# djamahl99/findnpropagate

Hardware: AMD Instinct MI355X
Metric: NuScenes scenes/s (30k pts, Transfusion voxel backbone) (higher is better)
Workload: dtype bf16

## Files before the change

findnpropagate_amd/csrc/spconv.hip:

```cpp
#include "rankgrid.h"
#include "sortedsweep.h"
#include "conv_launch.h"
#include <type_traits>

#ifndef FNP_ABLATE
#define FNP_ABLATE 0
#endif

namespace {

__device__ __forceinline__ float to_f32(float v) { return v; }
__device__ __forceinline__ float to_f32(__bf16 v) { return (float)v; }
__device__ __forceinline__ float to_f32(_Float16 v) { return (float)v; }
template <typename T> __device__ __forceinline__ T from_f32(float v);
template <> __device__ __forceinline__ float from_f32<float>(float v) { return v; }
template <> __device__ __forceinline__ __bf16 from_f32<__bf16>(float v) { return (__bf16)v; }
template <> __device__ __forceinline__ _Float16 from_f32<_Float16>(float v) { return (_Float16)v; }

template <typename TIn, typename TOut>
__global__ __launch_bounds__(256) void spconv_valu_kernel(const TIn *__restrict__ x, const TIn *__restrict__ w,
                                                          const int *__restrict__ nbr, int nbr_stride, int K,
                                                          const int *__restrict__ n_out, int cap,
                                                          TOut *__restrict__ y, const float *__restrict__ scale,
                                                          const float *__restrict__ shift,
                                                          const TOut *__restrict__ residual, int relu, int Cin, int Cout) {
    const int n = min(*n_out, cap);
    const long long total = (long long)n * Cout;
    for (long long t = (long long)blockIdx.x * blockDim.x + threadIdx.x; t < total; t += (long long)gridDim.x * blockDim.x) {
        const int row = (int)(t / Cout), co = (int)(t % Cout);
        float acc = 0.f;
        for (int k = 0; k < K; ++k) {
            const int idx = nbr[(size_t)k * nbr_stride + row];
            if (idx < 0) continue;
            const TIn *xr = x + (size_t)idx * Cin;
            const TIn *wr = w + ((size_t)k * Cout + co) * Cin;
            for (int ci = 0; ci < Cin; ++ci) acc = fmaf(to_f32(xr[ci]), to_f32(wr[ci]), acc);
        }
        float v = acc;
        if (scale) v = v * scale[co] + shift[co];
        if (residual) v = v + to_f32(residual[(size_t)row * Cout + co]);
        if (relu && v < 0.f) v = 0.f;
        y[(size_t)row * Cout + co] = from_f32<TOut>(v);
    }
}

template <int COUT, typename TOut>
__global__ __launch_bounds__(256) void spconv_first_kernel(const float *__restrict__ x, const float *__restrict__ w,
                                                           const int *__restrict__ nbr, int nbr_stride, int K,
                                                           const int *__restrict__ n_out, int cap,
                                                           TOut *__restrict__ y, const float *__restrict__ scale,
                                                           const float *__restrict__ shift,
                                                           const TOut *__restrict__ residual, int relu, int Cin) {
    extern __shared__ __attribute__((aligned(16))) unsigned char fnp_smem[];
    float *wl = reinterpret_cast<float *>(fnp_smem);
    for (int i = threadIdx.x; i < K * Cin * COUT; i += 256) {
        const int k = i / (Cin * COUT), r = i % (Cin * COUT);
        const int ci = r / COUT, co = r % COUT;
        wl[i] = w[((size_t)k * COUT + co) * Cin + ci];
    }
    __syncthreads();
    const int n = min(*n_out, cap);
    for (int row = blockIdx.x * 256 + threadIdx.x; row < n; row += gridDim.x * 256) {
        float acc[COUT];
#pragma unroll
        for (int co = 0; co < COUT; ++co) acc[co] = 0.f;
        for (int k0 = 0; k0 < K; k0 += 9) {
            int idx[9];
#pragma unroll
            for (int j = 0; j < 9; ++j) idx[j] = k0 + j < K ? nbr[(size_t)(k0 + j) * nbr_stride + row] : -1;
#pragma unroll
            for (int j = 0; j < 9; ++j) {
                if (k0 + j >= K) break;
                const bool ok = idx[j] >= 0;
                const float *xr = x + (size_t)(ok ? idx[j] : 0) * Cin;
                const float *wk = wl + (k0 + j) * Cin * COUT;
                float xv[8];
#pragma unroll
                for (int ci = 0; ci < 8; ++ci) xv[ci] = ci < Cin ? xr[ci] : 0.f;
#pragma unroll
                for (int ci = 0; ci < 8; ++ci) {
                    if (ci >= Cin) break;
                    const float xc = ok ? xv[ci] : 0.f;
#pragma unroll
                    for (int co = 0; co < COUT; ++co) acc[co] = fmaf(xc, wk[ci * COUT + co], acc[co]);
                }
            }
        }
#pragma unroll
        for (int co = 0; co < COUT; ++co) {
            float v = acc[co];
            if (scale) v = v * scale[co] + shift[co];
            if (residual) v = v + to_f32(residual[(size_t)row * COUT + co]);
            if (relu && v < 0.f) v = 0.f;
            y[(size_t)row * COUT + co] = from_f32<TOut>(v);
        }
    }
}

template <typename TOut>
int launch_first(const ConvArgs &a, int Cin) {
    const int grid = fnp_grid_for(a.cap, 256, 2048);
    const size_t lds = sizeof(float) * (size_t)a.K * Cin * 16;
    hipLaunchKernelGGL(HIP_KERNEL_NAME(spconv_first_kernel<16, TOut>), dim3(grid), dim3(256), lds, a.stream, (const float *)a.x,
                       (const float *)a.w, a.nbr, a.nbr_stride, a.K, a.n_out, a.cap, (TOut *)a.y, a.scale, a.shift, (const TOut *)a.residual,
                       a.relu, Cin);
    FNP_LAUNCH_CHECK();
    return FNP_OK;
}

template <int CIN, int COUT, int KVOL>
struct MfmaCfg {
    static constexpr bool PAIR = CIN == 16 && KVOL == 27;
    static constexpr int KEFF = PAIR ? (KVOL + 1) / 2 : KVOL;
    static constexpr int CH = PAIR ? 4 : CIN / 8;
    static constexpr int SLAB = COUT * CH;
    static constexpr int SW = (CH == 8 || CH == 4) ? 1 : 0;
    static constexpr bool ALLK = KVOL > 0 && (long long)KEFF * SLAB * 16 <= 65536;
    static constexpr int LDS_BYTES = (ALLK ? KEFF : 2) * SLAB * 16;
    static constexpr int KS = (CIN + 31) / 32;
    static constexpr int PFK = ALLK ? (KS == 1 ? 4 : 2) : 1;
    static constexpr int WH = 64;
    static constexpr int WZERO = 128;
    static constexpr int win_rows(int nw, int mb) { return nw * mb * 16 + 2 * WH; }
    static constexpr bool WIDE = COUT >= 32;
    static constexpr int ESTRIDE = COUT * 2 + 16;
    static constexpr int epi_sites(bool win) { return win ? 8 : 16; }
    static constexpr int epi_bytes(int nw, bool win, bool out16) { return (WIDE && out16 && !win) ? nw * epi_sites(win) * ESTRIDE : 0; }
    static constexpr int lds_bytes(int nw, int mb, bool win) { return LDS_BYTES + (win ? win_rows(nw, mb) * CH * 16 + WZERO : 0); }
};

template <int CIN, int COUT> struct MfmaWg {
    static constexpr int NW = (CIN == COUT && CIN >= 32) ? 8 : 4;
    static constexpr int MB = COUT >= 128 ? 3 : (CIN == COUT || (CIN == 16 && COUT == 32)) ? 2 : 4;
    static constexpr int MB_SMALL = 2;
};

template <int CIN, int COUT> struct MfmaOcc { static constexpr int WAVES = (CIN == 128 && COUT == 128) ? 2 : (CIN == COUT || (CIN == 16 && COUT == 32)) ? 4 : (CIN < COUT && COUT <= 64) ? 3 : 2; };

struct FusedRb {
    RG gi;
    int s[3], p[3];
    const int *out_coords;
    const unsigned *ell_rec;
    int ell_cap;
};

struct SplitOut {
    const void *addend;
    void *hi, *lo;
    int relu;
};

#ifdef FNP_MFMA_STAMP
__device__ unsigned long long g_mfma_stamps[8];
#define FNP_MS_NOW(v) do { __builtin_amdgcn_sched_barrier(0); asm volatile("s_memtime %0\n\ts_waitcnt lgkmcnt(0)" : "=s"(v)::"memory"); __builtin_amdgcn_sched_barrier(0); } while (0)
#define FNP_MS(ph) do { if (CIN == 128 && COUT == 128 && KVOL == 27) { unsigned long long n_; FNP_MS_NOW(n_); ms_acc[ph] += n_ - ms_prev; ms_prev = n_; } } while (0)
#else
#define FNP_MS(ph)
#endif
template <int CIN, int COUT, int NWO> struct NwOf { static constexpr int value = NWO ? NWO : MfmaWg<CIN, COUT>::NW; };
template <int CIN, int COUT, int MB, int KVOL, bool WIN, typename TOut, bool FUSED = false, typename TAct = __bf16, bool SORTED = false, int NWO = 0>
__global__ __launch_bounds__((NwOf<CIN, COUT, NWO>::value * 64), (MfmaOcc<CIN, COUT>::WAVES)) void spconv_mfma_kernel(const TAct *__restrict__ x, int x_bytes,
                                                             const TAct *__restrict__ w,
                                                             const int *__restrict__ nbr, int nbr_stride, int Krt,
                                                             const int *__restrict__ n_out, int cap,
                                                             TOut *__restrict__ y, const float *__restrict__ scale,
                                                             const float *__restrict__ shift,
                                                             const TOut *__restrict__ residual, int relu, int hints, FusedRb frb, SortedRb srb, SplitOut so) {
    using Cfg = MfmaCfg<CIN, COUT, KVOL>;
    constexpr int NWX = NwOf<CIN, COUT, NWO>::value;
    static_assert(!SORTED || (KVOL == 27 && !WIN && !FUSED && !Cfg::PAIR && !Cfg::ALLK), "sorted sweep: wide double-buffered 3x3x3 layers");
    using bf16x8 = typename Vec16<TAct>::v8;
    using bf16x4 = typename Vec16<TAct>::v4;
    static_assert(sizeof(TOut) == 4 || std::is_same<TOut, TAct>::value, "16-bit outputs have the activation type");
    static_assert(!FUSED || (KVOL == 27 && !WIN), "fused rulebook: 3x3x3 strided layers");
    constexpr int CH = Cfg::CH, SLAB = Cfg::SLAB, SW = Cfg::SW, KS = Cfg::KS, PFK = Cfg::PFK;
    constexpr bool ALLK = Cfg::ALLK;
    constexpr int WROWS = Cfg::win_rows(NWX, MB), WH = Cfg::WH;
    static_assert(!WIN || (CH == 8 && PFK == 1), "window path: 64 input channels, fragments read one offset ahead");
    constexpr int NB = COUT / 16;
    constexpr int NBH = NB < 4 ? NB : 4;
    constexpr int ROWS_PER_WAVE = MB * 16;
    constexpr int NW = NWX, NT = NW * 64;
    constexpr int ROWS_PER_WG = NW * ROWS_PER_WAVE;
    constexpr int NCH = (SLAB + NT - 1) / NT;
    constexpr int WST = (NCH + KS - 1) / KS;
    constexpr bool WDEEP = !ALLK && NCH <= 1;
    constexpr bool WD4 = !ALLK && (((NW == 8 || (NW == 4 && CIN == 128 && COUT == 64)) && NCH == KS && NCH == 4) || (NWO == 4 && NCH == 2 * KS && KS == 4) ||
                                   (NW == 4 && NCH == 2 * KS && KS == 2 && CIN == 64 && COUT == 128));
    constexpr int WDN = WD4 ? NCH / KS : 1;
    static_assert(CIN % 16 == 0 && COUT % 16 == 0, "channel counts must be multiples of 16");
    static_assert(ALLK || SLAB % NT == 0 || SLAB < NT, "unsupported slab size");

    extern __shared__ __attribute__((aligned(16))) unsigned char fnp_smem[];
    uint4 *wl = reinterpret_cast<uint4 *>(fnp_smem);
    unsigned char *const win = fnp_smem + Cfg::LDS_BYTES;
    constexpr unsigned WIN_ZERO = (unsigned)(Cfg::LDS_BYTES + WROWS * CH * 16);
    auto win_sw = [](unsigned d) -> unsigned { return (d >> 1) & 7u; };

    constexpr bool PAIR = Cfg::PAIR;
    constexpr bool GPAIR = !WIN && KS % 2 == 0 && PFK == 1;
    const int K = KVOL > 0 ? Cfg::KEFF : Krt;
    const int n = min(*n_out, cap);
    const int tid = threadIdx.x;
    const int lane = tid & 63, wave = tid >> 6;
    const int l15 = lane & 15, q = lane >> 4;
    const bool kvalid0 = PAIR || (q * 8) < CIN;
    const int qk = PAIR ? (q >> 1) : 0;

    const __amdgpu_buffer_rsrc_t xrsrc = __builtin_amdgcn_make_buffer_rsrc((void *)x, 0, x_bytes, 0x00020000);
    auto row_off = [&](int id) -> unsigned {
        return ((FNP_ABLATE & 1) || id < 0 || !kvalid0) ? 0x80000000u
                                                        : (unsigned)id * (unsigned)(CIN * 2) + (unsigned)(PAIR ? (q & 1) : q) * 16u;
    };
    auto gather = [&](unsigned roff, int ks) -> bf16x8 {
        u32x4 v = {0u, 0u, 0u, 0u};
        if (!(WIN && (FNP_ABLATE & 8))) v = __builtin_amdgcn_raw_buffer_load_b128(xrsrc, roff + (unsigned)ks * 64u, 0, 0);
        return *reinterpret_cast<bf16x8 *>(&v);
    };
    constexpr int SR = MB * 16;
    int *const fstrip = reinterpret_cast<int *>(fnp_smem + Cfg::lds_bytes(NWX, MB, WIN) +
                                                Cfg::epi_bytes(NWX, WIN, sizeof(TOut) == 2)) + wave * (27 * SR);
    int frow0 = 0;
    float *const ss_lds = reinterpret_cast<float *>(fnp_smem + Cfg::lds_bytes(NWX, MB, WIN) +
                                                    Cfg::epi_bytes(NWX, WIN, sizeof(TOut) == 2) +
                                                    (FUSED ? NWX * 27 * MB * 16 * 4 : 0));
    auto nbr_at = [&](int k, int r, int r_end) -> int {
        const int rc = r < r_end ? r : r_end - 1;
        const int kr = PAIR ? 2 * k + qk : k, KR = PAIR ? KVOL : K;
        const int kc = kr < KR ? kr : KR - 1;
        if constexpr (FUSED) return kr < KR ? fstrip[kc * SR + (r - frow0)] : -1;
        const int v = nbr[(FNP_ABLATE & 32) ? (size_t)((kc * 64 + rc) & 0x3fff) : (size_t)kc * nbr_stride + rc];
        return (r < r_end && kr < KR) ? v : -1;
    };
    auto nbr_raw = [&](int k, int r, int r_end) -> int {
        const int rc = r < r_end ? r : r_end - 1;
        const int kr = PAIR ? 2 * k + qk : k, KR = PAIR ? KVOL : K;
        const int kc = kr < KR ? kr : KR - 1;
        if (FNP_ABLATE & 512) return rc + kc - 13;
        if constexpr (FUSED) return fstrip[kc * SR + (r - frow0)];
        return nbr[(FNP_ABLATE & 32) ? (size_t)((kc * 64 + rc) & 0x3fff) : (size_t)kc * nbr_stride + rc];
    };
    auto k_live = [&](int k) -> bool { return PAIR ? (2 * k + qk < KVOL) : (k < K); };

    auto win_off = [&](int id, int wlo) -> unsigned {
        if (FNP_ABLATE & 64)
            return (unsigned)Cfg::LDS_BYTES + ((((unsigned)id << 6) & 0x3fc0u) ^ ((unsigned)q << 4));
        const unsigned d = (unsigned)(id - wlo);
        return d < (unsigned)WROWS ? (unsigned)Cfg::LDS_BYTES + ((d * CH + ((unsigned)q ^ win_sw(d))) << 4) : WIN_ZERO;
    };
    auto row_off_w = [&](int id, int wlo) -> unsigned {
        const unsigned d = (unsigned)(id - wlo);
        return ((FNP_ABLATE & 1) || id < 0 || d < (unsigned)WROWS) ? 0x80000000u
                                                                    : (unsigned)id * (unsigned)(CIN * 2) + (unsigned)q * 16u;
    };
    auto win_read = [&](unsigned off) -> u32x4 {
        if (FNP_ABLATE & 16) return u32x4{off, 0u, 0u, 0u};
        return *reinterpret_cast<const u32x4 *>(fnp_smem + off);
    };

    const int G = gridDim.x;
    const int xcd = blockIdx.x & 7, slot = blockIdx.x >> 3;
    const int per = G >> 3, rem = G & 7;
    const int range = (xcd < rem ? xcd * (per + 1) : rem * (per + 1) + (xcd - rem) * per) + slot;
    int row_begin, row_end;
    int xslots = 1;
    if constexpr (SORTED) {
        const XcdRows xr = fnp_xcd_rows(n, G, xcd);
        row_begin = xr.X0;
        row_end = xr.X1;
        xslots = xr.S;
    } else {
        fnp_range_rows(n, range, G, row_begin, row_end);
    }
    if (row_begin >= row_end) return;
    for (int c = tid; c < 2 * COUT; c += NWX * 64)
        ss_lds[c] = scale ? (c < COUT ? scale[c] : shift[c - COUT]) : (c < COUT ? 1.f : 0.f);

#define FNP_LDS_POS(row, chunk) ((row) * CH + ((chunk) ^ (((row) >> SW) & (CH - 1))))
    int aoff[KS];
#pragma unroll
    for (int ks = 0; ks < KS; ++ks) aoff[ks] = FNP_LDS_POS(l15, kvalid0 ? ks * 4 + q : (q & (CH - 1)));
    const int st_pos0 = FNP_LDS_POS(tid / CH, tid % CH);
    static_assert(SLAB < NT || ((NT / CH) % (CH << SW) == 0), "staging swizzle must be periodic in NT chunks");
    if (WIN && tid < Cfg::WZERO / 16) reinterpret_cast<uint4 *>(fnp_smem + WIN_ZERO)[tid] = make_uint4(0u, 0u, 0u, 0u);
    if (ALLK) {
        for (int p = tid; p < K * SLAB; p += NT) {
            const int kk = p / SLAB, r = p % SLAB;
            if constexpr (PAIR) {
                const int co = r / CH, c = r % CH, kr = 2 * kk + (c >> 1);
                uint4 v = make_uint4(0u, 0u, 0u, 0u);
                if (kr < KVOL) v = reinterpret_cast<const uint4 *>(w)[((size_t)kr * COUT + co) * 2 + (c & 1)];
                wl[kk * SLAB + FNP_LDS_POS(co, c)] = v;
            } else {
                wl[kk * SLAB + FNP_LDS_POS(r / CH, r % CH)] = reinterpret_cast<const uint4 *>(w)[p];
            }
        }
        __syncthreads();
    }

#ifdef FNP_MFMA_STAMP
    unsigned long long ms_acc[4] = {0, 0, 0, 0}, ms_prev;
    FNP_MS_NOW(ms_prev);
#endif
    bool first_tile = true;
// ... 379 lines not shown
                            *slot = bf16x4{(TAct)v[0], (TAct)v[1], (TAct)v[2], (TAct)v[3]};
                        }
                    }
#pragma unroll
                    for (int i = 0; i < NRD; ++i) {
                        const int r = rb + i * SPI + wsite;
                        int ro = r;
                        if constexpr (SORTED) ro = orow[mb][h][i];
                        const u32x4 t = *reinterpret_cast<const u32x4 *>(eb + (i * SPI + wsite) * ES + wchunk * 16);
                        if (r < row_end && !(FNP_ABLATE & 128)) {
                            *reinterpret_cast<u32x4 *>(y + (size_t)ro * COUT + wchunk * 8) = t;
                        }
                    }
                }
            }
        } else if constexpr (WIN && sizeof(TOut) == 2 && NB % 2 == 0) {
            const int poff = (q & 1) * 32 + (q >> 1) * 16;
#pragma unroll
            for (int mb = 0; mb < MBT; ++mb) {
                const int r = row0 + mb * 16 + l15;
                const bool live = r < row_end;
#pragma unroll
                for (int kp = 0; kp < NB / 2; ++kp) {
                    uint2 ra = make_uint2(0u, 0u), rb = make_uint2(0u, 0u);
                    if (residual && !(FNP_ABLATE & 256)) {
                        uint4 rv = make_uint4(0u, 0u, 0u, 0u);
                        if (live) rv = *reinterpret_cast<const uint4 *>(reinterpret_cast<const unsigned char *>(residual) + (size_t)r * (COUT * 2) + kp * 64 + poff);
                        auto t0 = __builtin_amdgcn_permlane16_swap(rv.x, rv.z, false, false);
                        auto t1 = __builtin_amdgcn_permlane16_swap(rv.y, rv.w, false, false);
                        ra = make_uint2(t0[0], t1[0]);
                        rb = make_uint2(t0[1], t1[1]);
                    }
                    uint2 o[2];
#pragma unroll
                    for (int h = 0; h < 2; ++h) {
                        const int nb = 2 * kp + h, c0 = nb * 16 + q * 4;
                        float v[4];
#pragma unroll
                        for (int j = 0; j < 4; ++j) v[j] = acc[nb][mb][j];
                        if (scale) {
                            const float4 s4 = *reinterpret_cast<const float4 *>(ss_lds + c0);
                            const float4 h4 = *reinterpret_cast<const float4 *>(ss_lds + COUT + c0);
                            v[0] = v[0] * s4.x + h4.x; v[1] = v[1] * s4.y + h4.y; v[2] = v[2] * s4.z + h4.z; v[3] = v[3] * s4.w + h4.w;
                        }
                        if (residual && !(FNP_ABLATE & 256)) {
                            const uint2 rr = h ? rb : ra;
                            const bf16x4 t = *reinterpret_cast<const bf16x4 *>(&rr);
#pragma unroll
                            for (int j = 0; j < 4; ++j) v[j] = v[j] + (float)t[j];
                        }
                        if (relu) {
#pragma unroll
                            for (int j = 0; j < 4; ++j) v[j] = v[j] < 0.f ? 0.f : v[j];
                        }
                        const bf16x4 ob = {(TAct)v[0], (TAct)v[1], (TAct)v[2], (TAct)v[3]};
                        o[h] = *reinterpret_cast<const uint2 *>(&ob);
                    }
                    auto t0 = __builtin_amdgcn_permlane16_swap(o[0].x, o[1].x, false, false);
                    auto t1 = __builtin_amdgcn_permlane16_swap(o[0].y, o[1].y, false, false);
                    if (live && !(FNP_ABLATE & 128))
                        *reinterpret_cast<uint4 *>(reinterpret_cast<unsigned char *>(y) + (size_t)r * (COUT * 2) + kp * 64 + poff) =
                            make_uint4(t0[0], t1[0], t0[1], t1[1]);
                }
            }
        } else {
#pragma unroll
        for (int nb = 0; nb < NB; ++nb) {
            const int c0 = nb * 16 + q * 4;
            float sc[4] = {1.f, 1.f, 1.f, 1.f}, sh[4] = {0.f, 0.f, 0.f, 0.f};
            if (scale) {
                const float4 s4 = *reinterpret_cast<const float4 *>(ss_lds + c0);
                const float4 h4 = *reinterpret_cast<const float4 *>(ss_lds + COUT + c0);
                sc[0] = s4.x; sc[1] = s4.y; sc[2] = s4.z; sc[3] = s4.w;
                sh[0] = h4.x; sh[1] = h4.y; sh[2] = h4.z; sh[3] = h4.w;
            }
#pragma unroll
            for (int mb = 0; mb < MBT; ++mb) {
                const int rpos = row0 + mb * 16 + l15;
                if (rpos >= row_end) continue;
                int r = rpos;
                if constexpr (SORTED) r = srb.perm[rpos];
                float v[4];
#pragma unroll
                for (int j = 0; j < 4; ++j) v[j] = scale ? acc[nb][mb][j] * sc[j] + sh[j] : acc[nb][mb][j];
                if (residual && !(FNP_ABLATE & 256)) {
                    const TOut *rp = residual + (size_t)r * COUT + c0;
#pragma unroll
                    for (int j = 0; j < 4; ++j) v[j] = v[j] + to_f32(rp[j]);
                }
                if (relu) {
#pragma unroll
                    for (int j = 0; j < 4; ++j) v[j] = v[j] < 0.f ? 0.f : v[j];
                }
                TOut *yp = y + (size_t)r * COUT + c0;
                if (FNP_ABLATE & 128) { if (v[0] == 12345.678f) yp[0] = from_f32<TOut>(v[1] + v[2] + v[3]); continue; }
                if constexpr (sizeof(TOut) == 2) {
                    bf16x4 o = {(TAct)v[0], (TAct)v[1], (TAct)v[2], (TAct)v[3]};
                    *reinterpret_cast<bf16x4 *>(yp) = o;
                } else {
                    if (so.hi) {
                        if (so.addend) {
                            const bf16x4 tv = *reinterpret_cast<const bf16x4 *>(reinterpret_cast<const TAct *>(so.addend) + (size_t)r * COUT + c0);
#pragma unroll
                            for (int j = 0; j < 4; ++j) v[j] = v[j] + (float)tv[j];
                        }
                        if (so.relu) {
#pragma unroll
                            for (int j = 0; j < 4; ++j) v[j] = v[j] < 0.f ? 0.f : v[j];
                        }
                        bf16x4 h, l;
#pragma unroll
                        for (int j = 0; j < 4; ++j) {
                            h[j] = (TAct)v[j];
                            l[j] = (TAct)(v[j] - (float)h[j]);
                        }
                        *reinterpret_cast<bf16x4 *>(reinterpret_cast<TAct *>(so.hi) + (size_t)r * COUT + c0) = h;
                        *reinterpret_cast<bf16x4 *>(reinterpret_cast<TAct *>(so.lo) + (size_t)r * COUT + c0) = l;
                    }
                    if (y) *reinterpret_cast<float4 *>(yp) = make_float4(v[0], v[1], v[2], v[3]);
                }
            }
        }
        }
        FNP_MS(3);
        first_tile = false;
    };
    int full, tper, tail_base, tstride = ROWS_PER_WG, tfirst = row_begin;
    if constexpr (SORTED) {
        const int round_rows = xslots * ROWS_PER_WG;
        full = (row_end - row_begin) / round_rows;
        tstride = round_rows;
        tfirst = row_begin + slot * ROWS_PER_WG;
        const int left0 = row_begin + full * round_rows;
        tper = fnp_tail_blocks(row_end - left0, xslots, NW);
        tail_base = left0 + slot * (NW * tper * 16);
        if (tail_base >= row_end) tper = 0;
    } else {
        const int nblk_wg = (row_end - row_begin + 15) >> 4;
        full = nblk_wg / (NW * MB);
        tper = (nblk_wg - full * NW * MB + NW - 1) / NW;
        tail_base = row_begin + full * ROWS_PER_WG;
    }
    if constexpr (SORTED) {
        const int rot = (xslots * 3 + 4) >> 3;
        for (int t = 0; t < full; ++t) run_tile(std::integral_constant<int, MB>{}, row_begin + t * tstride + ((slot + t * rot) % xslots) * ROWS_PER_WG);
    } else {
        for (int t = 0; t < full; ++t) run_tile(std::integral_constant<int, MB>{}, tfirst + t * tstride);
    }
    if (tper == MB) run_tile(std::integral_constant<int, MB>{}, tail_base);
    if constexpr (MB > 1) { if (tper == 1) run_tile(std::integral_constant<int, 1>{}, tail_base); }
    if constexpr (MB > 2) { if (tper == 2) run_tile(std::integral_constant<int, 2>{}, tail_base); }
    if constexpr (MB > 3) { if (tper == 3) run_tile(std::integral_constant<int, 3>{}, tail_base); }
#ifdef FNP_MFMA_STAMP
    if (CIN == 128 && COUT == 128 && KVOL == 27 && lane == 0)
        for (int ph = 0; ph < 4; ++ph) atomicAdd(&g_mfma_stamps[ph], ms_acc[ph]);
#endif
}

template <int CIN, int COUT, int KVOL, bool WIN, typename TOut, bool FUSED = false, int NWO = 0>
struct MfmaGeom {
    using Cfg = MfmaCfg<CIN, COUT, KVOL>;
    static constexpr int NWX = NwOf<CIN, COUT, NWO>::value;
    static constexpr int MB = NWO ? MfmaWg<CIN, COUT>::MB_SMALL : MfmaWg<CIN, COUT>::MB;
    static constexpr int lds = Cfg::lds_bytes(NWX, MB, WIN) + Cfg::epi_bytes(NWX, WIN, sizeof(TOut) == 2) +
                               (FUSED ? NWX * 27 * MB * 16 * 4 : 0) + COUT * 8;
    static constexpr int wg_regs = MfmaOcc<CIN, COUT>::WAVES * 4 / NWX;
    static constexpr int wg_per_cu = lds * wg_regs > 160 * 1024 ? 160 * 1024 / lds : wg_regs;
    static_assert(wg_per_cu >= 1 && lds * wg_per_cu <= 160 * 1024, "LDS budget of the resident workgroups");
    static int grid(int cap) {
        const int tiles = fnp_divup(cap, NWX * MB * 16);
        const int resident = 256 * wg_per_cu;
        const int fine = fnp_divup(cap, NWX * 16);
        return tiles >= resident ? resident : (fine < resident ? fine : resident);
    }
};
using SortedGeom = MfmaGeom<128, 128, 27, false, __bf16>;

template <int CIN, int COUT, int KVOL, bool WIN, typename TOut, bool FUSED = false, typename TAct = __bf16, bool SORTED = false, int NWO = 0>
int launch_mfma_k(const ConvArgs &a, const FusedRb *frb_in = nullptr, const SortedRb *srb_in = nullptr, const SplitOut *so_in = nullptr) {
    using Geom = MfmaGeom<CIN, COUT, KVOL, WIN, TOut, FUSED, NWO>;
    auto kern = spconv_mfma_kernel<CIN, COUT, Geom::MB, KVOL, WIN, TOut, FUSED, TAct, SORTED, NWO>;
    FusedRb frb{};
    if (FUSED) {
        if (!frb_in) return FNP_ERR_ARG;
        frb = *frb_in;
    }
    SortedRb srb{nullptr, nullptr};
    if (SORTED) {
        if (!srb_in || !srb_in->perm || !srb_in->blockmask) return FNP_ERR_ARG;
        srb = *srb_in;
    }
    if (Geom::lds > 64 * 1024) {
        static bool raised = false;
        if (const int rc = fnp_raise_lds(reinterpret_cast<const void *>(kern), Geom::lds, raised)) return rc;
    }
    hipLaunchKernelGGL(kern, dim3(Geom::grid(a.cap)), dim3(Geom::NWX * 64), Geom::lds, a.stream, (const TAct *)a.x, (int)a.x_bytes, (const TAct *)a.w,
                       a.nbr, a.nbr_stride, a.K, a.n_out, a.cap, (TOut *)a.y, a.scale, a.shift, (const TOut *)a.residual, a.relu, a.hints, frb, srb,
                       so_in ? *so_in : SplitOut{nullptr, nullptr, nullptr, 0});
    FNP_LAUNCH_CHECK();
    return FNP_OK;
}

template <int CIN, int COUT> struct HasWindow { static constexpr bool value = CIN == 64 && COUT == 64; };

template <int CIN, int COUT, typename TOut, typename TAct>
int launch_mfma(const ConvArgs &a, const SplitOut *so = nullptr) {
    if (a.K == 27) {
        if constexpr (HasWindow<CIN, COUT>::value) {
            if (a.hints & FNP_HINT_ROWS_RANKED) return launch_mfma_k<CIN, COUT, 27, true, TOut, false, TAct>(a, nullptr, nullptr, so);
        }
        if constexpr (CIN == 128 && COUT == 128 && sizeof(TOut) == 2) {
            if (a.cap < 256 * MfmaWg<CIN, COUT>::NW * MfmaWg<CIN, COUT>::MB * 16) return launch_mfma_k<CIN, COUT, 27, false, TOut, false, TAct, false, 4>(a);
        }
        return launch_mfma_k<CIN, COUT, 27, false, TOut, false, TAct>(a, nullptr, nullptr, so);
    }
    return launch_mfma_k<CIN, COUT, 0, false, TOut, false, TAct>(a, nullptr, nullptr, so);
}

template <typename TIn, typename TOut>
int launch_valu(const ConvArgs &a, int Cin, int Cout) {
    const int grid = fnp_grid_for((long long)a.cap * Cout, 256, 256 * 16);
    hipLaunchKernelGGL(HIP_KERNEL_NAME(spconv_valu_kernel<TIn, TOut>), dim3(grid), dim3(256), 0, a.stream, (const TIn *)a.x,
                       (const TIn *)a.w, a.nbr, a.nbr_stride, a.K, a.n_out, a.cap, (TOut *)a.y, a.scale, a.shift, (const TOut *)a.residual,
                       a.relu, Cin, Cout);
    FNP_LAUNCH_CHECK();
    return FNP_OK;
}

constexpr int kSortThreads = 1024, kSortQ = 16;
__global__ __launch_bounds__(256) void rowmask_kernel(const int *__restrict__ nbr, int nbr_stride, const int *__restrict__ n_out, int cap,
                                                      unsigned *__restrict__ rowmask) {
    const int n = min(*n_out, cap);
    for (int r = blockIdx.x * 256 + threadIdx.x; r < n; r += gridDim.x * 256) {
        unsigned m = 0u;
#pragma unroll
        for (int k = 0; k < 27; ++k) m |= (nbr[(size_t)k * nbr_stride + r] >= 0 ? 1u : 0u) << k;
        rowmask[r] = m;
    }
}
__global__ __launch_bounds__(kSortThreads) void classsort_place_kernel(const unsigned *__restrict__ rowmask, const int *__restrict__ n_out, int cap,
                                                                        int G, int tile_rows, int NW, int *__restrict__ perm,
                                                                        unsigned *__restrict__ blockmask) {
    constexpr int NWV = kSortThreads / 64;
    __shared__ unsigned long long wtot[NWV];
    const int n = min(*n_out, cap), tid = threadIdx.x, lane = tid & 63, wave = tid >> 6;
    const XcdRows xr = fnp_xcd_rows(n, G, blockIdx.y);
    if (xr.S == 0 || xr.X0 >= xr.X1) return;
    const int round_rows = xr.S * tile_rows, full = (xr.X1 - xr.X0) / round_rows;
    for (int i = blockIdx.x; i <= full; i += gridDim.x) {
        const int b = xr.X0 + i * round_rows, e = min(xr.X1, b + round_rows);
        if (b >= e) break;
        const int q = (e - b + kSortThreads - 1) / kSortThreads, r0 = b + tid * q;
        for (int j = (b >> 4) + tid; j < ((e + 15) >> 4); j += kSortThreads) blockmask[j] = 0u;
        unsigned m[kSortQ];
        unsigned long long cnt = 0ull;
#pragma unroll
        for (int u = 0; u < kSortQ; ++u) {
            m[u] = 0u;
            if (u < q && r0 + u < e) {
                m[u] = rowmask[r0 + u];
                cnt += 1ull << (16 * fnp_zclass(m[u]));
            }
        }
        unsigned long long v = cnt;
#pragma unroll
        for (int d = 1; d < 64; d <<= 1) {
            const unsigned long long t = __shfl_up(v, d);
            if (lane >= d) v += t;
        }
        if (lane == 63) wtot[wave] = v;
        __syncthreads();
        unsigned long long woff = 0ull, grand = 0ull;
#pragma unroll
        for (int wv = 0; wv < NWV; ++wv) {
            const unsigned long long t = wtot[wv];
            if (wv < wave) woff += t;
            grand += t;
        }
        const unsigned long long excl = v - cnt + woff;
        int run[4];
        const int t0 = (int)(grand & 0xffffu), t1 = (int)((grand >> 16) & 0xffffu), t2 = (int)((grand >> 32) & 0xffffu);
        run[0] = (int)(excl & 0xffffu);
        run[1] = t0 + (int)((excl >> 16) & 0xffffu);
        run[2] = t0 + t1 + (int)((excl >> 32) & 0xffffu);
        run[3] = t0 + t1 + t2 + (int)((excl >> 48) & 0xffffu);
#pragma unroll
        for (int u = 0; u < kSortQ; ++u) {
            if (u < q && r0 + u < e) {
                const int c = fnp_zclass(m[u]);
                const int pos = b + (c == 0 ? run[0]++ : c == 1 ? run[1]++ : c == 2 ? run[2]++ : run[3]++);
                perm[pos] = r0 + u;
                atomicOr(&blockmask[pos >> 4], m[u]);
            }
        }
        __syncthreads();
    }
}

#ifndef FNP_OUT128_MIN_CAP
#define FNP_OUT128_MIN_CAP (256 * 8 * 64)
#endif
constexpr int kOut128MinCap = FNP_OUT128_MIN_CAP;

template <typename TAct, typename TOut>
int dispatch_16(const ConvArgs &a, int Cin, int Cout, const SplitOut *so = nullptr) {
    const bool fits = fnp_fits32(a.x_bytes);
    if (fits && a.K == 3 && Cin == 128 && Cout == 128 && !a.residual && !so && a.cap >= kOut128MinCap)
        return fnp_launch_out128(std::is_same<TAct, __bf16>::value ? FNP_BF16 : FNP_F16, sizeof(TOut) == 4, a);
    int rc = FNP_ERR_ARG;
    if (fits && fnp_for_pair(Cin, Cout, rc, ConvPairs{}, [&](auto p) { return launch_mfma<decltype(p)::ci, decltype(p)::co, TOut, TAct>(a, so); })) return rc;
    if (so) return FNP_ERR_ARG;
    return launch_valu<TAct, TOut>(a, Cin, Cout);
}

bool fused_rb(const fnp_rankgrid *in_grid, const fnp_conv_geom *geom, const int *out_coords, FusedRb &frb) {
    if (!geom || !out_coords || !fnp_rg_valid(in_grid)) return false;
    for (int d = 0; d < 3; ++d)
        if (geom->ksize[d] != 3 || geom->stride[d] <= 0 || geom->padding[d] < 0) return false;
    if (in_grid->D != geom->in_shape[0] || in_grid->H != geom->in_shape[1] || in_grid->W != geom->in_shape[2]) return false;
    frb.gi = fnp_rg_view(in_grid);
    for (int d = 0; d < 3; ++d) {
        frb.s[d] = geom->stride[d];
        frb.p[d] = geom->padding[d];
    }
    frb.out_coords = out_coords;
    frb.ell_rec = nullptr;
    frb.ell_cap = 0;
    return true;
}

template <typename Pairs>
int launch_fused(const ConvArgs &a, int dtype, int Cin, int Cout, const FusedRb &frb, Pairs pairs) {
    int rc = FNP_ERR_ARG;
    fnp_for_pair(Cin, Cout, rc, pairs, [&](auto p) {
        return fnp_dispatch16(dtype, [&](auto t) {
            using T = typename decltype(t)::type;
            return launch_mfma_k<decltype(p)::ci, decltype(p)::co, 27, false, T, true, T>(a, &frb);
        });
    });
    return rc;
}

bool sorted_args_ok(const ConvArgs &a, int n_in_rows, const SortedRb &srb, int Cin, int Cout, bool need_y) {
    return fnp_conv_args_ok(a, n_in_rows, true, need_y) && srb.perm && srb.blockmask && Cin == 128 && Cout == 128 && fnp_fits32(a.x_bytes);
}

}

#ifdef FNP_MFMA_STAMP
extern "C" int fnp_debug_mfma_stamps(unsigned long long *out8) {
    if (hipMemcpyFromSymbol(out8, HIP_SYMBOL(g_mfma_stamps), sizeof(unsigned long long) * 8) != hipSuccess) return FNP_ERR_HIP;
    unsigned long long zero[8] = {0};
    if (hipMemcpyToSymbol(HIP_SYMBOL(g_mfma_stamps), zero, sizeof(zero)) != hipSuccess) return FNP_ERR_HIP;
    return FNP_OK;
}
#endif

int fnp_spconv_forward_f32_mfma(const ConvArgs &a, int wperm, int Cin, int Cout);

extern "C" int fnp_spconv_forward(const void *feat_in, int in_dtype, int n_in_rows, const void *weight, const int *nbr,
                                  int nbr_stride, int K, const int *n_out, int cap_out, void *feat_out, int out_dtype,
                                  const float *scale, const float *shift, const void *residual, int relu, int hints,
                                  int Cin, int Cout, fnp_stream_t stream) {
    const ConvArgs a{feat_in, (long long)n_in_rows * Cin * (in_dtype == FNP_F32 ? 4 : 2), weight, nbr, nbr_stride, K, n_out, cap_out, feat_out,
                     scale, shift, residual, relu, hints, (hipStream_t)stream};
    if (!fnp_conv_args_ok(a, n_in_rows) || K <= 0 || Cin <= 0 || Cout <= 0) return FNP_ERR_ARG;
    if (in_dtype == FNP_F32) {
        if (Cout == 16 && Cin <= 8 && (size_t)K * Cin * 16 * 4 <= 60000) {
            if (out_dtype == FNP_F32) return launch_first<float>(a, Cin);
            if (out_dtype == FNP_BF16) return launch_first<__bf16>(a, Cin);
            if (out_dtype == FNP_F16) return launch_first<_Float16>(a, Cin);
            return FNP_ERR_ARG;
        }
        if (out_dtype == FNP_F32 && !(hints & FNP_HINT_VALU)) {
            const int rc = fnp_spconv_forward_f32_mfma(a, (hints & FNP_HINT_W_PERMUTED) != 0, Cin, Cout);
            if (rc != FNP_ERR_ARG) return rc;
        }
        if (hints & FNP_HINT_W_PERMUTED) return FNP_ERR_ARG;
        if (out_dtype == FNP_F32) return launch_valu<float, float>(a, Cin, Cout);
        if (out_dtype == FNP_BF16) return launch_valu<float, __bf16>(a, Cin, Cout);
        if (out_dtype == FNP_F16) return launch_valu<float, _Float16>(a, Cin, Cout);
        return FNP_ERR_ARG;
    }
    return fnp_dispatch16(in_dtype, [&](auto t) {
        using T = typename decltype(t)::type;
        if (out_dtype == in_dtype) return dispatch_16<T, T>(a, Cin, Cout);
        if (out_dtype == FNP_F32) return dispatch_16<T, float>(a, Cin, Cout);
        return (int)FNP_ERR_ARG;
    });
}

extern "C" int fnp_spconv_forward_split(const void *feat_in, int in_dtype, int n_in_rows, const void *weight, const int *nbr, int nbr_stride,
                                        int K, const int *n_out, int cap_out, float *feat_out, const float *scale, const float *shift,
                                        const float *residual, const void *addend, int relu, int hints, int Cin, int Cout, void *out_hi,
                                        void *out_lo, fnp_stream_t stream) {
    const ConvArgs a{feat_in, (long long)n_in_rows * Cin * 2, weight, nbr, nbr_stride, K, n_out, cap_out, feat_out, scale, shift, residual, 0, hints,
                     (hipStream_t)stream};
    if (!fnp_conv_args_ok(a, n_in_rows, true, false) || !out_hi || !out_lo || K <= 0 || Cin <= 0 || Cout <= 0)
        return FNP_ERR_ARG;
    if (!fnp_aligned(7, out_hi, out_lo, addend) || !fnp_aligned(15, feat_out)) return FNP_ERR_ARG;
    const SplitOut so{addend, out_hi, out_lo, relu};
    return fnp_dispatch16(in_dtype, [&](auto t) { return dispatch_16<typename decltype(t)::type, float>(a, Cin, Cout, &so); });
}

extern "C" int fnp_spconv_forward_strided(const void *feat_in, int in_dtype, int n_in_rows, const void *weight,
                                          const fnp_rankgrid *in_grid, const fnp_conv_geom *geom, const int *out_coords,
                                          const int *n_out, int cap_out, void *feat_out, int out_dtype, const float *scale,
                                          const float *shift, int relu, int Cin, int Cout, fnp_stream_t stream) {
    const ConvArgs a{feat_in, (long long)n_in_rows * Cin * 2, weight, nullptr, cap_out, 27, n_out, cap_out, feat_out, scale, shift, nullptr, relu, 0,
                     (hipStream_t)stream};
    FusedRb frb;
    if (!fnp_conv_args_ok(a, n_in_rows, false) || out_dtype != in_dtype || !fnp_fits32(a.x_bytes) || !fused_rb(in_grid, geom, out_coords, frb))
        return FNP_ERR_ARG;
    return launch_fused(a, in_dtype, Cin, Cout, frb, PairList<ChPair<16, 32>, ChPair<32, 64>, ChPair<64, 128>>{});
}

extern "C" int fnp_spconv_forward_ell_mfma(const void *feat_in, int in_dtype, int n_in_rows, const void *weight, const void *records, int cap_rows,
                                           int pool_records, const int *n_out, void *feat_out, int out_dtype, const float *scale, const float *shift,
                                           const void *residual, int relu, int Cin, int Cout, fnp_stream_t stream) {
    const ConvArgs a{feat_in, (long long)n_in_rows * Cin * 2, weight, nullptr, cap_rows, 27, n_out, cap_rows, feat_out, scale, shift, residual, relu, 0,
                     (hipStream_t)stream};
    if (!fnp_conv_args_ok(a, n_in_rows, false) || !records || pool_records < 0 || !fnp_aligned(15, records) || out_dtype != in_dtype) return FNP_ERR_ARG;
    if (!fnp_fits32(a.x_bytes) || (long long)cap_rows + pool_records >= (1ll << 26) || n_in_rows >= (1 << 27)) return FNP_ERR_ARG;
    FusedRb frb{};
    frb.ell_rec = (const unsigned *)records;
    frb.ell_cap = cap_rows;
    return launch_fused(a, in_dtype, Cin, Cout, frb, PairList<ChPair<16, 16>, ChPair<16, 32>>{});
}


extern "C" long long fnp_classsort_workspace_bytes(int cap_out) {
    if (cap_out <= 0) return 0;
    return (long long)cap_out * 4;
}

extern "C" int fnp_rulebook_classsort(const int *nbr, int nbr_stride, int K, const unsigned *rowmask, const int *n_out, int cap_out, int Cin,
                                      int Cout, int *perm, unsigned *blockmask, void *workspace, long long workspace_bytes,
                                      fnp_stream_t stream) {
    if (!n_out || !perm || !blockmask || K != 27 || cap_out <= 0) return FNP_ERR_ARG;
    if (Cin != 128 || Cout != 128) return FNP_ERR_ARG;
    hipStream_t s = (hipStream_t)stream;
    if (!rowmask) {
        if (!nbr || nbr_stride < cap_out || !workspace) return FNP_ERR_ARG;
        if (workspace_bytes < fnp_classsort_workspace_bytes(cap_out)) return FNP_ERR_WORKSPACE;
        hipLaunchKernelGGL(rowmask_kernel, dim3(fnp_grid_for(cap_out, 256)), dim3(256), 0, s, nbr, nbr_stride, n_out, cap_out, (unsigned *)workspace);
        FNP_LAUNCH_CHECK();
        rowmask = (const unsigned *)workspace;
    }
    const int grid = SortedGeom::grid(cap_out);
    constexpr int NW = SortedGeom::NWX, TILE = NW * SortedGeom::MB * 16;
    const int slots = (grid >> 3) + ((grid & 7) ? 1 : 0);
    if ((long long)slots * TILE > (long long)kSortThreads * kSortQ) return FNP_ERR_ARG;
    const int rounds = fnp_divup(fnp_divup(cap_out, 8) + 16 * (slots + 1), (long long)((grid >> 3) > 0 ? (grid >> 3) : 1) * TILE) + 1;
    hipLaunchKernelGGL(classsort_place_kernel, dim3(rounds < 1024 ? rounds : 1024, 8), dim3(kSortThreads), 0, s, rowmask, n_out, cap_out, grid, TILE, NW, perm,
                       blockmask);
    FNP_LAUNCH_CHECK();
    return FNP_OK;
}

extern "C" int fnp_spconv_forward_sorted(const void *feat_in, int dtype, int n_in_rows, const void *weight, const int *nbr, int nbr_stride,
                                         const int *perm, const unsigned *blockmask, const int *n_out, int cap_out, void *feat_out,
                                         const float *scale, const float *shift, const void *residual, int relu, int Cin, int Cout,
                                         fnp_stream_t stream) {
    const ConvArgs a{feat_in, (long long)n_in_rows * Cin * 2, weight, nbr, nbr_stride, 27, n_out, cap_out, feat_out, scale, shift, residual, relu, 0,
                     (hipStream_t)stream};
    const SortedRb srb{perm, blockmask};
    if (!sorted_args_ok(a, n_in_rows, srb, Cin, Cout, true)) return FNP_ERR_ARG;
    static_assert(SortedGeom::NWX == kSortedNW && SortedGeom::MB == kSortedMB && MfmaOcc<128, 128>::WAVES == 2,
                  "the row pipeline sweeps the sorted grid's tiles: its geometry is the one sortedsweep.h names");
    if ((dtype == FNP_BF16 || dtype == FNP_F16) && cap_out >= 256 * kSortedNW * 16) return fnp_launch_rows128(dtype, a, perm, blockmask, SortedGeom::grid(cap_out));
    return fnp_dispatch16(dtype, [&](auto t) {
        using T = typename decltype(t)::type;
        return launch_mfma_k<128, 128, 27, false, T, false, T, true>(a, nullptr, &srb);
    });
}

extern "C" int fnp_spconv_forward_sorted_split(const void *feat_in, int dtype, int n_in_rows, const void *weight, const int *nbr, int nbr_stride,
                                               const int *perm, const unsigned *blockmask, const int *n_out, int cap_out, float *feat_out,
                                               const float *scale, const float *shift, const float *residual, const void *addend, int relu,
                                               int Cin, int Cout, void *out_hi, void *out_lo, fnp_stream_t stream) {
    const ConvArgs a{feat_in, (long long)n_in_rows * Cin * 2, weight, nbr, nbr_stride, 27, n_out, cap_out, feat_out, scale, shift, residual, 0, 0,
                     (hipStream_t)stream};
    const SortedRb srb{perm, blockmask};
    if (!sorted_args_ok(a, n_in_rows, srb, Cin, Cout, false) || !out_hi || !out_lo) return FNP_ERR_ARG;
    if (!fnp_aligned(7, out_hi, out_lo, addend) || !fnp_aligned(15, feat_out)) return FNP_ERR_ARG;
    using Geom32 = MfmaGeom<128, 128, 27, false, float>;
    static_assert(Geom32::NWX == SortedGeom::NWX && Geom32::MB == SortedGeom::MB && Geom32::wg_per_cu == SortedGeom::wg_per_cu,
                  "the f32-output sweep has the grid of the 16-bit one at every capacity");
    const SplitOut so{addend, out_hi, out_lo, relu};
    return fnp_dispatch16(dtype, [&](auto t) {
        return launch_mfma_k<128, 128, 27, false, float, false, typename decltype(t)::type, true>(a, nullptr, &srb, &so);
    });
}
```

Baseline: 13940.

## Add dedicated persistent MFMA kernel for strided 64-to-128 downsample conv

```diff
diff --git a/findnpropagate_amd/csrc/down128.h b/findnpropagate_amd/csrc/down128.h
--- /dev/null
+++ b/findnpropagate_amd/csrc/down128.h
@@ -0,0 +1,11 @@
+#pragma once
+#include "conv_launch.h"
+#include "rankgrid.h"
+
+struct Down128Rb {
+    RG gi;
+    int s[3], p[3];
+    const int *out_coords;
+};
+
+__attribute__((visibility("hidden"))) int fnp_launch_down128(int dtype, const ConvArgs &a, int n_in_rows, const Down128Rb &rb);
diff --git a/findnpropagate_amd/csrc/spconv.hip b/findnpropagate_amd/csrc/spconv.hip
--- a/findnpropagate_amd/csrc/spconv.hip
+++ b/findnpropagate_amd/csrc/spconv.hip
@@ -1,6 +1,7 @@
 #include "rankgrid.h"
 #include "sortedsweep.h"
 #include "conv_launch.h"
+#include "down128.h"
 #include <type_traits>
 
 #ifndef FNP_ABLATE
@@ -986,6 +987,15 @@
 #endif
 constexpr int kOut128MinCap = FNP_OUT128_MIN_CAP;
 
+#ifndef FNP_DOWN128_MIN_CAP
+#define FNP_DOWN128_MIN_CAP (256 * 8 * 32)
+#endif
+#ifdef FNP_DOWN128_OFF
+constexpr int kDown128MinCap = 0x7fffffff;
+#else
+constexpr int kDown128MinCap = FNP_DOWN128_MIN_CAP;
+#endif
+
 template <typename TAct, typename TOut>
 int dispatch_16(const ConvArgs &a, int Cin, int Cout, const SplitOut *so = nullptr) {
     const bool fits = fnp_fits32(a.x_bytes);
@@ -1096,6 +1106,10 @@
     FusedRb frb;
     if (!fnp_conv_args_ok(a, n_in_rows, false) || out_dtype != in_dtype || !fnp_fits32(a.x_bytes) || !fused_rb(in_grid, geom, out_coords, frb))
         return FNP_ERR_ARG;
+    if (Cin == 64 && Cout == 128 && cap_out >= kDown128MinCap) {
+        Down128Rb drb{frb.gi, {frb.s[0], frb.s[1], frb.s[2]}, {frb.p[0], frb.p[1], frb.p[2]}, frb.out_coords};
+        return fnp_launch_down128(in_dtype, a, n_in_rows, drb);
+    }
     return launch_fused(a, in_dtype, Cin, Cout, frb, PairList<ChPair<16, 32>, ChPair<32, 64>, ChPair<64, 128>>{});
 }
 
diff --git a/findnpropagate_amd/csrc/spconv_down128.hip b/findnpropagate_amd/csrc/spconv_down128.hip
--- /dev/null
+++ b/findnpropagate_amd/csrc/spconv_down128.hip
@@ -0,0 +1,269 @@
+#include "down128.h"
+#include "sortedsweep.h"
+#include <type_traits>
+
+#ifndef FNP_D128_ABLATE
+#define FNP_D128_ABLATE 0
+#endif
+
+namespace {
+
+__device__ uint4 g_down128_zero[8];
+
+template <int I> __device__ __forceinline__ int d128_row_share(int v) { return __builtin_amdgcn_update_dpp(0, v, 0x150 + I, 0xf, 0xf, false); }
+template <int I, int N, typename F> __device__ __forceinline__ void d128_static_for(F &&f) {
+    if constexpr (I < N) {
+        f(std::integral_constant<int, I>{});
+        d128_static_for<I + 1, N>(f);
+    }
+}
+typedef __attribute__((address_space(1))) const void *d128_gptr;
+typedef __attribute__((address_space(3))) void *d128_lptr;
+
+#define D128_VMCNT(N) asm volatile("s_waitcnt vmcnt(%0)" ::"n"(N) : "memory")
+#define D128_LGKMCNT0() asm volatile("s_waitcnt lgkmcnt(0)" ::: "memory")
+
+constexpr int kD128NW = 8, kD128MB = 3, kD128NT = kD128NW * 64, kD128K = 27;
+constexpr int kD128Slab = 128 * 128, kD128Ring = 3;
+constexpr int kD128RowBuf = kD128MB * 16 * 128;
+constexpr int kD128RowsOff = kD128Ring * kD128Slab;
+constexpr int kD128SsOff = kD128RowsOff + 2 * kD128NW * kD128RowBuf;
+constexpr int kD128Lds = kD128SsOff + 2 * 128 * 4;
+static_assert(kD128Lds == 145 * 1024 && kD128Lds <= 160 * 1024, "slab ring + two row buffers per wave + scale / shift");
+static_assert(2 * kD128RowBuf >= 16 * (128 * 2 + 16), "the epilogue's transpose strip aliases the wave's row buffers");
+
+template <typename TAct>
+__global__ __launch_bounds__(kD128NT, 2) void spconv_down128_kernel(const TAct *__restrict__ x, int n_in, const TAct *__restrict__ w, const int *__restrict__ n_out,
+                                                                    int cap, TAct *__restrict__ y, const float *__restrict__ scale,
+                                                                    const float *__restrict__ shift, int relu, Down128Rb frb) {
+    using bf16x8 = typename Vec16<TAct>::v8;
+    using bf16x4 = typename Vec16<TAct>::v4;
+    constexpr int C = 128, NB = 8, NBH = 4, NW = kD128NW, MB = kD128MB, ROWS_PER_WG = NW * MB * 16, K = kD128K;
+    constexpr int NSLAB = (FNP_D128_ABLATE & 2) ? 0 : 2;
+    extern __shared__ __attribute__((aligned(16))) unsigned char fnp_smem[];
+    const int n = min(*n_out, cap);
+    const int tid = threadIdx.x, lane = tid & 63, wave = __builtin_amdgcn_readfirstlane(tid >> 6);
+    const int l15 = lane & 15, q = lane >> 4;
+    const int r8 = lane >> 3, c8 = lane & 7;
+    unsigned char *const rowbuf = fnp_smem + kD128RowsOff + wave * (2 * kD128RowBuf);
+
+    const int G = gridDim.x, xcd = blockIdx.x & 7, slot = blockIdx.x >> 3;
+    const XcdRows xr = fnp_xcd_rows(n, G, xcd);
+    const int row_begin = xr.X0, row_end = xr.X1, xslots = xr.S;
+    if (row_begin >= row_end) return;
+    float *const ss_lds = reinterpret_cast<float *>(fnp_smem + kD128SsOff);
+    if (tid < 2 * C) ss_lds[tid] = scale ? (tid < C ? scale[tid] : shift[tid - C]) : (tid < C ? 1.f : 0.f);
+
+    unsigned foff[2];
+#pragma unroll
+    for (int ksl = 0; ksl < 2; ++ksl) foff[ksl] = (unsigned)l15 * 128u + ((unsigned)((ksl * 4 + q) ^ ((l15 >> 1) & 7)) << 4);
+    unsigned wsrc[2];
+#pragma unroll
+    for (int j = 0; j < 2; ++j) {
+        const int wr = (j * 8 + wave) * 8 + r8;
+        wsrc[j] = (unsigned)wr * 128u + ((unsigned)(c8 ^ ((wr >> 1) & 7)) << 4);
+    }
+    auto dma_slab_piece = [&](int koffset, int ring, int j) {
+        const unsigned char *wk = reinterpret_cast<const unsigned char *>(w) + (size_t)koffset * kD128Slab;
+        unsigned ws = wsrc[j];
+        asm volatile("" : "+v"(ws));
+        __builtin_amdgcn_global_load_lds((d128_gptr)(wk + ws), (d128_lptr)(fnp_smem + ring * kD128Slab + (j * 8 + wave) * 1024), 16, 0, 0);
+    };
+
+    struct Ent {
+        int e[K];
+    };
+    const int c16 = lane & 15, r4 = lane >> 4;
+    auto tile_epos = [&](int tile_base, int mbt) -> int { return tile_base + wave * (mbt * 16) + 8 * (c16 >> 1) + 2 * r4 + (c16 & 1); };
+    auto load_coords = [&](int tile_base, int mbt) -> int4 {
+        return reinterpret_cast<const int4 *>(frb.out_coords)[min(tile_epos(tile_base, mbt), row_end - 1)];
+    };
+    auto resolve = [&](const int4 c) -> Ent {
+        Ent r;
+        nbr_row<3, 3, 3>(frb.gi, c.x, c.y * frb.s[0] - frb.p[0], c.z * frb.s[1] - frb.p[1], c.w * frb.s[2] - frb.p[2], r.e, 1);
+        return r;
+    };
+
+    auto run_tile = [&](auto mbt_tag, const int tile_base, const Ent ent, const int next_base, const int next_mbt) __attribute__((always_inline)) -> Ent {
+        constexpr int MBT = decltype(mbt_tag)::value, NI = MBT * 2;
+        constexpr int NROW = (FNP_D128_ABLATE & 4) ? 0 : NI;
+        const int row0 = tile_base + wave * (MBT * 16);
+        const bool ehas = c16 < 2 * NI && tile_epos(tile_base, MBT) < row_end;
+        auto dma_row_piece = [&](int ev, auto half_tag, auto ic) {
+            constexpr int half = decltype(half_tag)::value, ii = decltype(ic)::value;
+            const int e0 = d128_row_share<2 * ii>(ev), e1 = d128_row_share<2 * ii + 1>(ev);
+            const int er = (FNP_D128_ABLATE & 8) ? -1 : (lane & 8) ? e1 : e0;
+            const int sw = ((ii & 1) << 2) | (r8 >> 1);
+            const unsigned char *src = (unsigned)er < (unsigned)n_in ? reinterpret_cast<const unsigned char *>(x) + (size_t)er * 128 + ((c8 ^ sw) << 4)
+                                                                     : reinterpret_cast<const unsigned char *>(g_down128_zero) + (c8 << 4);
+            __builtin_amdgcn_global_load_lds((d128_gptr)src, (d128_lptr)(rowbuf + half * kD128RowBuf + ii * 1024), 16, 0, 0);
+        };
+        auto dma_piece = [&](auto pc, auto half_tag, const int k, const int ev, const int ring_k2) {
+            constexpr int p = decltype(pc)::value;
+            if constexpr (p < NROW) dma_row_piece(ev, half_tag, pc);
+            else if constexpr (p < NROW + NSLAB) dma_slab_piece(k + 2, ring_k2, p - NROW);
+        };
+        bf16x8 xb[2][MBT];
+        auto read_xb = [&](int half, int k) {
+            const unsigned char *rb = rowbuf + half * kD128RowBuf;
+#pragma unroll
+            for (int ksl = 0; ksl < 2; ++ksl)
+#pragma unroll
+                for (int mb = 0; mb < MBT; ++mb) {
+                    u32x4 t = u32x4{(unsigned)k, 0u, 0u, 0u};
+                    if (!(FNP_D128_ABLATE & 4)) t = *reinterpret_cast<const u32x4 *>(rb + mb * 2048 + foff[ksl]);
+                    xb[ksl][mb] = *reinterpret_cast<const bf16x8 *>(&t);
+                }
+        };
+
+        f32x4 acc[NB][MBT];
+#pragma unroll
+        for (int nb = 0; nb < NB; ++nb)
+#pragma unroll
+            for (int mb = 0; mb < MBT; ++mb) acc[nb][mb] = (f32x4){0.f, 0.f, 0.f, 0.f};
+
+        auto step = [&](auto half_tag, auto more_tag, auto last_tag, const int k, const int e_next, const int ring_k, const int ring_k2) __attribute__((always_inline)) {
+            constexpr int half = decltype(half_tag)::value;
+            constexpr bool more = decltype(more_tag)::value, last = decltype(last_tag)::value;
+            constexpr int NG = 4, SLOTS = NG * MBT, NP = NROW + NSLAB;
+            const unsigned char *wk = fnp_smem + ring_k * kD128Slab;
+            const int ev = ehas ? e_next : -1;
+            bf16x8 wa[2][NBH];
+            auto read_wa = [&](auto gc) {
+                constexpr int g = decltype(gc)::value;
+#pragma unroll
+                for (int j = 0; j < NBH; ++j) {
+                    u32x4 t = u32x4{(unsigned)k, 1u, 0u, 0u};
+                    if (!(FNP_D128_ABLATE & 2)) t = *reinterpret_cast<const u32x4 *>(wk + ((g & 1) * NBH + j) * 2048 + foff[g >> 1]);
+                    wa[g & 1][j] = *reinterpret_cast<const bf16x8 *>(&t);
+                }
+            };
+            read_wa(std::integral_constant<int, 0>{});
+            D128_LGKMCNT0();
+            __builtin_amdgcn_sched_barrier(0);
+            d128_static_for<0, NG>([&](auto gc) {
+                constexpr int g = decltype(gc)::value;
+                if constexpr (g + 1 < NG) read_wa(std::integral_constant<int, g + 1>{});
+                d128_static_for<0, MBT>([&](auto mc) {
+                    constexpr int mb = decltype(mc)::value, sl = g * MBT + mb;
+#pragma unroll
+                    for (int j = 0; j < NBH; ++j) {
+                        if (FNP_D128_ABLATE & 1) asm volatile("" ::"v"(wa[g & 1][j]), "v"(xb[g >> 1][mb]));
+                        else acc[(g & 1) * NBH + j][mb] = mfma16(wa[g & 1][j], xb[g >> 1][mb], acc[(g & 1) * NBH + j][mb]);
+                    }
+                    if constexpr (more) {
+                        d128_static_for<sl * NP / SLOTS, (sl + 1) * NP / SLOTS>([&](auto pc) { dma_piece(pc, half_tag, k, ev, ring_k2); });
+                    }
+                    __builtin_amdgcn_sched_barrier(0);
+                });
+            });
+            if constexpr (more) D128_VMCNT(NROW + NSLAB);
+            else D128_VMCNT(0);
+            if constexpr (!last) read_xb(half ^ 1, k);
+            __builtin_amdgcn_sched_barrier(0);
+            __builtin_amdgcn_s_barrier();
+            __builtin_amdgcn_sched_barrier(0);
+        };
+        using H0 = std::integral_constant<int, 0>;
+        using H1 = std::integral_constant<int, 1>;
+
+        D128_LGKMCNT0();
+        D128_VMCNT(0);
+        __builtin_amdgcn_sched_barrier(0);
+        {
+            const int ev0 = ehas ? ent.e[0] : -1, ev1 = ehas ? ent.e[1] : -1;
+            d128_static_for<0, NROW>([&](auto ic) { dma_row_piece(ev0, H0{}, ic); });
+            d128_static_for<0, NSLAB>([&](auto jc) { dma_slab_piece(0, 0, decltype(jc)::value); });
+            d128_static_for<0, NROW>([&](auto ic) { dma_row_piece(ev1, H1{}, ic); });
+            d128_static_for<0, NSLAB>([&](auto jc) { dma_slab_piece(1, 1, decltype(jc)::value); });
+        }
+        __builtin_amdgcn_sched_barrier(0);
+        D128_VMCNT(NROW + NSLAB);
+        read_xb(0, 0);
+        __builtin_amdgcn_sched_barrier(0);
+        __builtin_amdgcn_s_barrier();
+        __builtin_amdgcn_sched_barrier(0);
+
+        int4 nc = make_int4(0, 0, 0, 0);
+        d128_static_for<0, K>([&](auto kc) {
+            constexpr int k = decltype(kc)::value;
+            constexpr bool more = k + 2 < K, last = k + 1 == K;
+            if constexpr (k == K - 2) {
+                if (next_mbt) nc = load_coords(next_base, next_mbt);
+            }
+            step(std::integral_constant<int, (k & 1)>{}, std::integral_constant<bool, more>{}, std::integral_constant<bool, last>{}, k,
+                 more ? ent.e[more ? k + 2 : 0] : 0, k % 3, (k + 2) % 3);
+        });
+
+        constexpr int EH = 16, LPR = C / 8, SPI = 64 / LPR, NRD = EH / SPI, ES = C * 2 + 16;
+        unsigned char *const eb = rowbuf;
+        int lane_e = lane;
+        asm volatile("" : "+v"(lane_e));
+        const int l15 = lane_e & 15, q = lane_e >> 4;
+        const int wsite = lane_e / LPR, wchunk = lane_e % LPR;
+#pragma unroll
+        for (int mb = 0; mb < MBT; ++mb) {
+            const int rb = row0 + mb * 16;
+#pragma unroll
+            for (int nb = 0; nb < NB; ++nb) {
+                const int c0 = nb * 16 + q * 4;
+                float v[4];
+#pragma unroll
+                for (int j = 0; j < 4; ++j) v[j] = acc[nb][mb][j];
+                if (scale) {
+                    const float4 s4 = *reinterpret_cast<const float4 *>(ss_lds + c0);
+                    const float4 h4 = *reinterpret_cast<const float4 *>(ss_lds + C + c0);
+                    v[0] = v[0] * s4.x + h4.x; v[1] = v[1] * s4.y + h4.y; v[2] = v[2] * s4.z + h4.z; v[3] = v[3] * s4.w + h4.w;
+                }
+                if (relu) {
+#pragma unroll
+                    for (int j = 0; j < 4; ++j) v[j] = v[j] < 0.f ? 0.f : v[j];
+                }
+                *reinterpret_cast<bf16x4 *>(eb + l15 * ES + c0 * 2) = bf16x4{(TAct)v[0], (TAct)v[1], (TAct)v[2], (TAct)v[3]};
+            }
+#pragma unroll
+            for (int i = 0; i < NRD; ++i) {
+                const int r = rb + i * SPI + wsite;
+                const u32x4 t = *reinterpret_cast<const u32x4 *>(eb + (i * SPI + wsite) * ES + wchunk * 16);
+                if (r < row_end) *reinterpret_cast<u32x4 *>(y + (size_t)r * C + wchunk * 8) = t;
+            }
+        }
+        Ent nent = ent;
+        if (next_mbt) nent = resolve(nc);
+        return nent;
+    };
+
+    const int round_rows = xslots * ROWS_PER_WG;
+    const int full = (row_end - row_begin) / round_rows;
+    const int left0 = row_begin + full * round_rows;
+    int tper = fnp_tail_blocks(row_end - left0, xslots, NW);
+    const int tail_base = left0 + slot * (NW * tper * 16);
+    if (tail_base >= row_end) tper = 0;
+    auto full_base = [&](int t) -> int { return row_begin + t * round_rows + slot * ROWS_PER_WG; };
+    if (full == 0 && tper == 0) return;
+    Ent ent = resolve(load_coords(full ? full_base(0) : tail_base, full ? MB : tper));
+    for (int t = 0; t < full; ++t) {
+        const bool last = t + 1 == full;
+        ent = run_tile(std::integral_constant<int, MB>{}, full_base(t), ent, last ? tail_base : full_base(t + 1), last ? tper : MB);
+    }
+    if (tper == 3) run_tile(std::integral_constant<int, 3>{}, tail_base, ent, 0, 0);
+    if (tper == 2) run_tile(std::integral_constant<int, 2>{}, tail_base, ent, 0, 0);
+    if (tper == 1) run_tile(std::integral_constant<int, 1>{}, tail_base, ent, 0, 0);
+}
+
+template <typename TAct>
+int launch_down128(const ConvArgs &a, int n_in_rows, const Down128Rb &rb) {
+    auto kern = spconv_down128_kernel<TAct>;
+    static bool raised = false;
+    if (const int rc = fnp_raise_lds(reinterpret_cast<const void *>(kern), kD128Lds, raised)) return rc;
+    hipLaunchKernelGGL(kern, dim3(256), dim3(kD128NT), kD128Lds, a.stream, (const TAct *)a.x, n_in_rows, (const TAct *)a.w, a.n_out, a.cap, (TAct *)a.y, a.scale,
+                       a.shift, a.relu, rb);
+    FNP_LAUNCH_CHECK();
+    return FNP_OK;
+}
+
+}
+
+int fnp_launch_down128(int dtype, const ConvArgs &a, int n_in_rows, const Down128Rb &rb) {
+    return fnp_dispatch16(dtype, [&](auto t) { return launch_down128<typename decltype(t)::type>(a, n_in_rows, rb); });
+}
```

Result: slower. 13800 (-1.0%).
